# yizuo417/RollingDepth

Hardware: AMD Instinct MI355X
Metric: depth frames/sec at 768px snip_len=3, 1-step denoise; 1/2/4/8 MI355X (higher is better)
Workload: dtype f16; 1 GPU; fast preset: 100-frame 768x768 video, dilations [1, 25] (cap_dilation=True), snippet_len 3, 1-step DDIM, aligner 2000 it, refine 0; SD2-shaped UNet+VAE random-init; preset=fast, frames=100, res=768, parallelism=snippet-dp1

## Files before the change

### include/rdmi.h

```cpp
#ifndef RDMI_H
#define RDMI_H

#include <stddef.h>

#ifdef __cplusplus
extern "C" {
#endif

#define RDMI_OK 0
#define RDMI_E_ARG 1001
#define RDMI_E_ALIGN 1002
#define RDMI_E_UNSUPPORTED 1003

#define RDMI_F16 0
#define RDMI_F32 1
#define RDMI_U8 2
#define RDMI_F32_X3 3
#define RDMI_F32_X6 4

#define RDMI_RESIZE_NEAREST 0
#define RDMI_RESIZE_BILINEAR 1
#define RDMI_RESIZE_BICUBIC 2

#define RDMI_EPI_NONE 0
#define RDMI_EPI_GEGLU 1
#define RDMI_EPI_SILU 2

const char* rdmi_last_error(void);
int rdmi_version(void);

typedef struct rdmi_gemm_args {
  const void* A; long lda; long strideA;
  const void* W; long ldw; long strideW;
  void* C; long ldc; long strideC; int c_f32;
  const float* bias;
  const void* residual; long ldr; long strideR;
  const float* rowbias; int rows_per_group; long rowbias_ld;
  float alpha;
  int M, N, K, batch;
  int epilogue;
  float* gn_part; long gn_ld;
  int dtype;
} rdmi_gemm_args;
int rdmi_gemm(const rdmi_gemm_args* args, void* stream);

typedef struct rdmi_conv_args {
  const void* x; const void* w; void* y;
  const float* bias; const void* residual; const float* rowbias;
  int B, H, W, Cin, Cout, kh, kw, stride, pad_top, pad_left, upsample, Ho, Wo, Kp;
  long y_ld; long res_ld; float alpha; long rowbias_ld;
  float* gn_part; long gn_ld;
  const float* in_mean_rstd; const float* in_gamma; const float* in_beta; int in_groups, in_silu;
  int dtype;
  const void* w_up2;
  const float* in_affine;
} rdmi_conv_args;
int rdmi_conv2d(const rdmi_conv_args* args, void* stream);
int rdmi_conv2d_in_gn_supported(const rdmi_conv_args* args);

long rdmi_groupnorm_workspace(int B, int G);
int rdmi_groupnorm_stats(const void* x, int dtype, int B, long HW, int C, int G, float eps,
                         float* mean_rstd, float* workspace, void* stream);
int rdmi_groupnorm_stats_partials(const float* part, long part_ld, int B, long HW, int C, int G, float eps,
                                  float* mean_rstd, void* stream);
int rdmi_groupnorm_affine(const float* mean_rstd, const float* gamma, const float* beta, int B, int C, int G,
                          float* out, void* stream);
int rdmi_groupnorm_apply(const void* x, void* y, int dtype, int B, long HW, int C, int G,
                         const float* mean_rstd, const float* gamma, const float* beta, int silu,
                         void* stream);

long rdmi_conv3x3_to1_gn_workspace(int B, int H, int W);
int rdmi_conv3x3_to1_gn(const void* x, int dtype, int B, int H, int W, int C, int G, const float* mean_rstd,
                        const float* gamma, const float* beta, int silu, const float* w, float bias,
                        void* y, int y_dtype, float* workspace, void* stream);

int rdmi_layernorm(const void* x, void* y, int dtype, long M, int C, const float* gamma, const float* beta,
                   float eps, void* stream);

int rdmi_attention_fwd(const void* q, const void* k, const void* v, void* o, int B, int H, int Sq,
                       int Sk, int D, long q_ld, long k_ld, long v_ld, long o_ld, long q_bs,
                       long k_bs, long v_bs, long o_bs, float scale, int dtype, void* stream);

int rdmi_attention_smallkv(const void* q, const void* k, const void* v, void* o, int B, int H,
                           int Sq, int L, int D, long q_ld, long o_ld, long q_bs, long o_bs,
                           long kv_bs, float scale, int dtype, void* stream);

int rdmi_cross_attn_pair(const void* x, void* y, long M, int C, int H, const float* ln_gamma,
                         const float* ln_beta, float eps, const float* w, const float* u, const float* c,
                         void* stream);

int rdmi_softmax_rows(const float* s, void* p, long rows, long cols, long p_ld, float scale, int p_dtype,
                      void* stream);

int rdmi_nchw_to_nhwc(const void* x, int x_f32, void* y, int y_dtype, int B, int C, int H, int W, int Cpad,
                      float scale, long x_bstride, long x_cstride, void* stream);
int rdmi_nhwc_to_nchw_f32(const void* x, int dtype, long ld, float* y, int B, int C, int H, int W,
                          float scale, float shift, void* stream);
int rdmi_concat_channels(const void* a, int Ca, const void* b, int Cb, void* y, long P, int dtype, void* stream);
int rdmi_resize_nearest(const void* x, int B, int H, int W, int C, void* y, int Ho, int Wo, int dtype,
                        void* stream);
int rdmi_transpose(const void* src, void* dst, int batch, long rows, long cols, long src_ld,
                   long dst_ld, int dtype, void* stream);
int rdmi_gather_unet_input(const void* rgb, long rgb_frame_ld, const void* depth,
                           long depth_frame_ld, int depth_bcast, const int* frame_idx, int count,
                           long HW, void* out, int dtype, void* stream);
int rdmi_ddim_combine(const void* x, long ld_x, const void* e, long ld_e, void* y, long ld_y,
                      long P, int C, int Cpad, float ca, float cb, float out_scale, long e_period,
                      int dtype, void* stream);
int rdmi_snippet_average(const void* src, int n, int w, int stride, int N, long P, int C, int ld,
                         void* out, int dtype, void* stream);
int rdmi_colorize(const void* depth, int dtype, long n, const void* minmax, const unsigned char* lut, int lut_n,
                  unsigned char* rgb, int* index, void* stream);
int rdmi_snippet_accumulate(const void* src, int dtype, int k0, int nloc, int w, int stride, int N, long P, int C,
                            int ld, double* sum, void* stream);
int rdmi_snippet_finish(const double* sum, int n, int w, int stride, int N, long P, int C, int ld, void* out,
                        int dtype, void* stream);
int rdmi_snippet_average_strided(const void* src, int n, int w, int stride, int start_step, int N, long P, int C,
                                 int ld, void* out, int dtype, void* stream);
int rdmi_snippet_accumulate_strided(const void* src, int dtype, int k0, int nloc, int w, int stride, int start_step,
                                    int N, long P, int C, int ld, double* sum, void* stream);
int rdmi_snippet_finish_strided(const double* sum, int n, int w, int stride, int start_step, int N, long P, int C,
                                int ld, void* out, int dtype, void* stream);
int rdmi_minmax(const void* x, int x_f32, long n, float* minmax, float* workspace, void* stream);
int rdmi_renormalize_f32(float* x, long n, const float* minmax, void* stream);

typedef struct rdmi_aligner_args {
  int n_dil;
// ... 139 lines not shown
```

### rollingdepth_amd/_native.py

```python
from __future__ import annotations

import ctypes as C
import os

_LIB_PATH = os.environ.get("RDMI_LIB") or os.path.join(os.path.dirname(os.path.abspath(__file__)), "_lib", "librdmi.so")

vp = C.c_void_p
i32 = C.c_int
i64 = C.c_long
f32 = C.c_float


class GemmArgs(C.Structure):
    _fields_ = [
        ("A", vp), ("lda", i64), ("strideA", i64),
        ("W", vp), ("ldw", i64), ("strideW", i64),
        ("C", vp), ("ldc", i64), ("strideC", i64), ("c_f32", i32),
        ("bias", vp),
        ("residual", vp), ("ldr", i64), ("strideR", i64),
        ("rowbias", vp), ("rows_per_group", i32), ("rowbias_ld", i64),
        ("alpha", f32),
        ("M", i32), ("N", i32), ("K", i32), ("batch", i32),
        ("epilogue", i32),
        ("gn_part", vp), ("gn_ld", i64),
        ("dtype", i32),
    ]


class ConvArgs(C.Structure):
    _fields_ = [
        ("x", vp), ("w", vp), ("y", vp),
        ("bias", vp), ("residual", vp), ("rowbias", vp),
        ("B", i32), ("H", i32), ("W", i32), ("Cin", i32), ("Cout", i32), ("kh", i32), ("kw", i32),
        ("stride", i32), ("pad_top", i32), ("pad_left", i32), ("upsample", i32), ("Ho", i32), ("Wo", i32),
        ("Kp", i32),
        ("y_ld", i64), ("res_ld", i64), ("alpha", f32), ("rowbias_ld", i64),
        ("gn_part", vp), ("gn_ld", i64),
        ("in_mean_rstd", vp), ("in_gamma", vp), ("in_beta", vp), ("in_groups", i32), ("in_silu", i32),
        ("dtype", i32),
        ("w_up2", vp),
        ("in_affine", vp),
    ]


class AlignerArgs(C.Structure):
    _fields_ = [
        ("n_dil", i32),
        ("x", vp * 8), ("s", vp * 8), ("t", vp * 8),
        ("n", i32 * 8), ("stride", i32 * 8),
        ("w", i32 * 8), ("seq_len", i32), ("P", i64),
        ("lr", f32), ("beta1", f32), ("beta2", f32), ("eps", f32), ("lmda2", f32), ("lmda3", f32),
        ("depth_w", f32), ("loss_scale", f32),
        ("iters", i32),
        ("history", vp), ("workspace", vp),
        ("start_step", i32 * 8),
    ]


_SIGS = {
    "rdmi_last_error": (C.c_char_p, []),
    "rdmi_version": (i32, []),
    "rdmi_gemm": (i32, [C.POINTER(GemmArgs), vp]),
    "rdmi_conv2d": (i32, [C.POINTER(ConvArgs), vp]),
    "rdmi_conv2d_in_gn_supported": (i32, [C.POINTER(ConvArgs)]),
    "rdmi_groupnorm_workspace": (i64, [i32, i32]),
    "rdmi_groupnorm_stats": (i32, [vp, i32, i32, i64, i32, i32, f32, vp, vp, vp]),
    "rdmi_groupnorm_stats_partials": (i32, [vp, i64, i32, i64, i32, i32, f32, vp, vp]),
    "rdmi_groupnorm_apply": (i32, [vp, vp, i32, i32, i64, i32, i32, vp, vp, vp, i32, vp]),
    "rdmi_conv3x3_to1_gn_workspace": (i64, [i32, i32, i32]),
    "rdmi_conv3x3_to1_gn": (i32, [vp, i32, i32, i32, i32, i32, i32, vp, vp, vp, i32, vp, f32, vp, i32, vp, vp]),
    "rdmi_layernorm": (i32, [vp, vp, i32, i64, i32, vp, vp, f32, vp]),
    "rdmi_attention_fwd": (i32, [vp, vp, vp, vp, i32, i32, i32, i32, i32, i64, i64, i64, i64, i64, i64, i64, i64,
                                 f32, i32, vp]),
    "rdmi_attention_smallkv": (i32, [vp, vp, vp, vp, i32, i32, i32, i32, i32, i64, i64, i64, i64, i64, f32, i32, vp]),
    "rdmi_cross_attn_pair": (i32, [vp, vp, i64, i32, i32, vp, vp, f32, vp, vp, vp, vp]),
    "rdmi_softmax_rows": (i32, [vp, vp, i64, i64, i64, f32, i32, vp]),
    "rdmi_nchw_to_nhwc": (i32, [vp, i32, vp, i32, i32, i32, i32, i32, i32, f32, i64, i64, vp]),
    "rdmi_nhwc_to_nchw_f32": (i32, [vp, i32, i64, vp, i32, i32, i32, i32, f32, f32, vp]),
    "rdmi_concat_channels": (i32, [vp, i32, vp, i32, vp, i64, i32, vp]),
    "rdmi_resize_nearest": (i32, [vp, i32, i32, i32, i32, vp, i32, i32, i32, vp]),
    "rdmi_transpose": (i32, [vp, vp, i32, i64, i64, i64, i64, i32, vp]),
    "rdmi_gather_unet_input": (i32, [vp, i64, vp, i64, i32, vp, i32, i64, vp, i32, vp]),
    "rdmi_ddim_combine": (i32, [vp, i64, vp, i64, vp, i64, i64, i32, i32, f32, f32, f32, i64, i32, vp]),
    "rdmi_snippet_average": (i32, [vp, i32, i32, i32, i32, i64, i32, i32, vp, i32, vp]),
    "rdmi_snippet_accumulate": (i32, [vp, i32, i32, i32, i32, i32, i32, i64, i32, i32, vp, vp]),
    "rdmi_snippet_finish": (i32, [vp, i32, i32, i32, i32, i64, i32, i32, vp, i32, vp]),
    "rdmi_snippet_average_strided": (i32, [vp, i32, i32, i32, i32, i32, i64, i32, i32, vp, i32, vp]),
    "rdmi_snippet_accumulate_strided": (i32, [vp, i32, i32, i32, i32, i32, i32, i32, i64, i32, i32, vp, vp]),
    "rdmi_snippet_finish_strided": (i32, [vp, i32, i32, i32, i32, i32, i64, i32, i32, vp, i32, vp]),
    "rdmi_colorize": (i32, [vp, i32, i64, vp, vp, i32, vp, vp, vp]),
    "rdmi_resize_workspace": (C.c_size_t, [i32, i32, i32, i32, i32, i32]),
    "rdmi_attention_d512": (i32, [vp, vp, vp, vp, i32, i32, i32, i32] + [i64] * 8 + [C.c_float, vp, vp]),
    "rdmi_resize": (i32, [vp, i32, i64, i64, i64, i64, i32, i32, i32, i32, i32, i32, i32, i32, vp, vp, vp]),
    "rdmi_minmax": (i32, [vp, i32, i64, vp, vp, vp]),
    "rdmi_renormalize_f32": (i32, [vp, i64, vp, vp]),
    "rdmi_aligner_workspace": (i64, [C.POINTER(AlignerArgs)]),
    "rdmi_aligner_optimize": (i32, [C.POINTER(AlignerArgs), vp]),
    "rdmi_aligner_prepare": (i32, [vp, i32, i32, i32, i32, i32, i32, i32, vp, vp, vp]),
    "rdmi_aligner_merge": (i32, [i32, C.POINTER(vp), i32, C.POINTER(vp), C.POINTER(vp), C.POINTER(i32),
                                 C.POINTER(i32), C.POINTER(i32), i32, i64, vp, vp, vp]),
    "rdmi_aligner_merge_strided": (i32, [i32, C.POINTER(vp), i32, C.POINTER(vp), C.POINTER(vp), C.POINTER(i32),
                                         C.POINTER(i32), C.POINTER(i32), C.POINTER(i32), i32, i64, vp, vp, vp]),
    "rdmi_groupnorm_affine": (i32, [vp, vp, vp, i32, i32, i32, vp, vp]),
    "rdmi_aligner_merge_partial_window": (i32, [i32, C.POINTER(vp), i32, C.POINTER(vp), C.POINTER(vp),
                                                C.POINTER(i32), C.POINTER(i32), C.POINTER(i32), C.POINTER(i32),
                                                C.POINTER(i32), i32, i32, i64, vp, vp, vp]),
    "rdmi_aligner_merge_finish_pieces": (i32, [i32, C.POINTER(i32), C.POINTER(i32), C.POINTER(i32), i32, i32, i64,
                                               i32, C.POINTER(i32), C.POINTER(i32), vp, vp, vp]),
    "rdmi_aligner_merge_partial_window_strided": (i32, [i32, C.POINTER(vp), i32, C.POINTER(vp), C.POINTER(vp),
                                                        C.POINTER(i32), C.POINTER(i32), C.POINTER(i32),
                                                        C.POINTER(i32), C.POINTER(i32), C.POINTER(i32), i32, i32, i32,
                                                        i64, vp, vp, vp]),
    "rdmi_aligner_merge_finish_pieces_strided": (i32, [i32, C.POINTER(i32), C.POINTER(i32), C.POINTER(i32),
                                                       C.POINTER(i32), i32, i32, i32, i64, i32, C.POINTER(i32),
                                                       C.POINTER(i32), vp, vp, vp]),
    "rdmi_aligner_merge_moments": (i32, [i32, C.POINTER(vp), i32, C.POINTER(vp), C.POINTER(vp), C.POINTER(i32),
                                         C.POINTER(i32), C.POINTER(i32), C.POINTER(i32), i32, i64, vp, vp, vp, vp]),
    "rdmi_aligner_merge_partial_window_moments": (i32, [i32, C.POINTER(vp), i32, C.POINTER(vp), C.POINTER(vp),
                                                        C.POINTER(i32), C.POINTER(i32), C.POINTER(i32),
                                                        C.POINTER(i32), C.POINTER(i32), C.POINTER(i32), i32, i32, i32,
                                                        i64, vp, vp, vp]),
    "rdmi_aligner_merge_finish_pieces_moments": (i32, [i32, C.POINTER(i32), C.POINTER(i32), C.POINTER(i32),
                                                       C.POINTER(i32), i32, i32, i32, i64, i32, C.POINTER(i32),
                                                       C.POINTER(i32), vp, vp, vp, vp]),
    "rdmi_scale_spread_f32": (i32, [vp, i64, vp, vp]),
    "rdmi_aligner_merge_median": (i32, [i32, C.POINTER(vp), i32, C.POINTER(vp), C.POINTER(vp), C.POINTER(i32),
                                        C.POINTER(i32), C.POINTER(i32), C.POINTER(i32), i32, i64, vp, vp, vp, vp]),
    "rdmi_aligner_merge_partial_window_terms": (i32, [i32, C.POINTER(vp), i32, C.POINTER(vp), C.POINTER(vp),
                                                      C.POINTER(i32), C.POINTER(i32), C.POINTER(i32),
                                                      C.POINTER(i32), C.POINTER(i32), C.POINTER(i32), i32, i32, i32,
                                                      i64, vp, vp, i64, vp, vp]),
    "rdmi_aligner_median_rows": (i32, [vp, i64, vp, vp, i32, i64, i32, vp, vp, vp]),
    "rdmi_depth_metrics_workspace": (i64, [i32, i64]),
    "rdmi_depth_moments": (i32, [vp, i32, vp, i32, vp, i32, i64, f32, f32, vp, vp]),
    "rdmi_depth_fit": (i32, [vp, i32, i64, i32, vp, vp, vp]),
    "rdmi_depth_errors": (i32, [vp, i32, vp, i32, vp, i32, i64, f32, f32, vp, f32, f32, vp, vp, vp]),
    "rdmi_depth_moments_space": (i32, [vp, i32, vp, i32, vp, i32, i64, f32, f32, i32, vp, vp]),
    "rdmi_depth_errors_space": (i32, [vp, i32, vp, i32, vp, i32, i64, f32, f32, vp, i32, f32, f32, vp, vp, vp]),
    "rdmi_depth_temporal": (i32, [vp, i32, vp, i32, vp, vp, vp, i32, i32, i32, i32, f32, f32, vp, i32, f32, f32, vp,
                                  vp, vp]),
    "rdmi_select_bins": (i32, []),
    "rdmi_select_passes": (i32, []),
    "rdmi_select_state_bytes": (i64, []),
    "rdmi_quantiles_workspace": (i64, []),
    "rdmi_select_hist": (i32, [vp, i32, vp, i64, vp, i32, i32, vp, vp]),
# ... 47 lines not shown
```

### rollingdepth_amd/csrc/conv_occ2.hip

```cpp
#include "gemm_kernels.h"

namespace rdmi_gk {

template <int MODE>
static void occ2_mode_launch(bool gn, bool pipe, dim3 g, hipStream_t s, const GemmP& p) {
  if (gn && pipe)
    hipLaunchKernelGGL((conv_halo_occ2_kernel<MODE, true, true>), g, dim3(256), 0, s, p);
  else if (gn)
    hipLaunchKernelGGL((conv_halo_occ2_kernel<MODE, true, false>), g, dim3(256), 0, s, p);
  else if (pipe)
    hipLaunchKernelGGL((conv_halo_occ2_kernel<MODE, false, true>), g, dim3(256), 0, s, p);
  else
    hipLaunchKernelGGL((conv_halo_occ2_kernel<MODE, false, false>), g, dim3(256), 0, s, p);
}

void launch_conv_occ2(int mode, bool gn, bool pipe, dim3 g, hipStream_t s, const GemmP& p) {
  if (mode == 3) {
    if (pipe)
      hipLaunchKernelGGL((conv_halo_occ2_kernel<3, false, true>), g, dim3(256), 0, s, p);
    else
      hipLaunchKernelGGL((conv_halo_occ2_kernel<3, false, false>), g, dim3(256), 0, s, p);
  } else if (mode == 2)
    occ2_mode_launch<2>(gn, pipe, g, s, p);
  else
    occ2_mode_launch<1>(gn, pipe, g, s, p);
}

void launch_conv_h32(bool gn, dim3 g, hipStream_t s, const GemmP& p) {
  if (gn)
    hipLaunchKernelGGL((conv_halo32_kernel<true>), g, dim3(256), 0, s, p);
  else
    hipLaunchKernelGGL((conv_halo32_kernel<false>), g, dim3(256), 0, s, p);
}

void launch_gemm_occ2(int bn, dim3 g, hipStream_t s, const GemmP& p) {
  if (bn == 160 && !p.geglu)
    hipLaunchKernelGGL((gemm_occ2_kernel<0, 160>), g, dim3(256), 0, s, p);
  else
    hipLaunchKernelGGL((gemm_occ2_kernel<0, 128>), g, dim3(256), 0, s, p);
}

}
```

### rollingdepth_amd/csrc/gemm.hip

```cpp
#include "gemm_kernels.h"

#include <stdlib.h>

namespace {

using namespace rdmi_gk;


int occ2_mode() {
  const char* e = getenv("RDMI_GEMM_OCC2");
  return e ? atoi(e) : 1;
}

int pp_mode() {
  const char* e = getenv("RDMI_GEMM_PP");
  return e ? atoi(e) : 1;
}

double tile_cost(long tiles, int bm, int bn, double eff) {
  return (double)((tiles + 255) / 256) * bm * bn / eff;
}

template <int MODE, int WM, int RN>
void launch_pp(const GemmP& p, int batch, hipStream_t s) {
  constexpr int BM = WM * 128, BN = (8 / WM) * RN * 16;
  dim3 g(p.N / BN, rdmi::div_up(p.M, BM), batch);
  static_assert(RN == 4, "ping-pong tiles use RN = 4");
  launch_gemm_pp(MODE, WM, 0, g, s, p);
}

template <int MODE>
void launch_mode(const GemmP& p, int batch, hipStream_t s, bool force128) {
  if (MODE == 0) {
    const int oc = occ2_mode();
    const bool pick = !p.geglu && batch == 1 && !p.c_f32 && p.N <= 1920 && p.N % 128 != 0;
    if (oc == 2 || (oc == 1 && pick)) {
      const char* e160 = getenv("RDMI_GEMM_BN160");
      const int bn = (p.N % 160 == 0 && !p.geglu && !(e160 && e160[0] == '0')) ? 160 : 128;
      dim3 g(rdmi::div_up(p.N, bn), rdmi::div_up(p.M, 128), batch);
      launch_gemm_occ2(bn, g, s, p);
      return;
    }
  }
  const int pp = pp_mode();
  if (pp != 0 && (MODE == 0 || p.cmaj)) {
    const char* dbg = MODE == 0 ? getenv("RDMI_GEMM_DBG") : nullptr;
    if (dbg && p.N % 256 == 0) {
      dim3 g(p.N / 256, rdmi::div_up(p.M, 256), batch);
      const int dv = atoi(dbg);
      if (dv == 1 || dv == 5 || dv == 8 || dv == 12) {
        launch_gemm_pp(0, 2, dv, g, s, p);
        return;
      }
    }
    const long mt256 = rdmi::div_up(p.M, 256), mt512 = rdmi::div_up(p.M, 512);
    const long ct = rdmi::div_up(p.N, 128);
    const double classic = tile_cost(mt256 * ct * batch, 256, 128, 1.0);
    double best = pp == 2 ? 1e300 : classic;
    int pick = 0;
    if (p.N % 256 == 0) {
      const double c = tile_cost(mt256 * (p.N / 256) * batch, 256, 256, 1.3);
      if (c < best) best = c, pick = 1;
    }
    if (p.N % 128 == 0) {
      const double c = tile_cost(mt512 * (p.N / 128) * batch, 512, 128, 1.1);
      if (c < best) best = c, pick = 3;
    }
    switch (pick) {
      case 1: launch_pp<MODE, 2, 4>(p, batch, s); return;
      case 3: launch_pp<MODE, 4, 4>(p, batch, s); return;
      default: break;
    }
  }
  const long mt256 = (p.M + 255) / 256;
  if (force128 || p.N % 128 == 0 || p.N > 512) {
    if (mt256 * ((p.N + 127) / 128) * batch >= 512) {
      dim3 g(rdmi::div_up(p.N, 128), rdmi::div_up(p.M, 256), batch);
      launch_gemm_classic(MODE, 256, 128, g, s, p);
    } else {
      dim3 g(rdmi::div_up(p.N, 128), rdmi::div_up(p.M, 128), batch);
      launch_gemm_classic(MODE, 128, 128, g, s, p);
    }
  } else {
    dim3 g(rdmi::div_up(p.N, 64), rdmi::div_up(p.M, 256), batch);
    launch_gemm_classic(MODE, 256, 64, g, s, p);
  }
}

int launch(GemmP p, int batch, hipStream_t s, bool force128, int mode) {
  const char* gm = getenv("RDMI_GEMM_GROUP");
  p.group_m = gm ? atoi(gm) : 8;
  if (mode == 2)
    launch_mode<2>(p, batch, s, force128);
  else if (mode == 1)
    launch_mode<1>(p, batch, s, force128);
  else
    launch_mode<0>(p, batch, s, force128);
  return rdmi::check_launch("gemm");
}

bool al16(const void* p) { return ((uintptr_t)p & 15) == 0; }

bool vec_ok(const GemmP& p) {
  const uintptr_t csz = p.c_f32 ? 16 : 8;
  bool ok = p.ldc % 4 == 0 && p.sC % 4 == 0 && ((uintptr_t)p.C % csz) == 0;
  if (p.R) ok = ok && p.ldr % 4 == 0 && p.sR % 4 == 0 && ((uintptr_t)p.R & 7) == 0;
  if (p.bias) ok = ok && ((uintptr_t)p.bias & 15) == 0;
  if (p.rowbias) ok = ok && ((uintptr_t)p.rowbias & 15) == 0 && p.rb_ld % 4 == 0;
  return ok;
}

int halo_mode() {
  const char* he = getenv("RDMI_CONV_HALO");
  return he ? atoi(he) : 3;
}

bool halo_eligible(const rdmi_conv_args* a, int hmode) {
  return hmode != 0 && a->kh == 3 && a->kw == 3 && a->Cin % 64 == 0 && a->stride == 1 && a->pad_top == 1 &&
         a->pad_left == 1 && a->Ho % 16 == 0 && a->Wo % 16 == 0 && a->Cout % 64 == 0 &&
         a->Ho == (a->upsample ? 2 * a->H : a->H) && a->Wo == (a->upsample ? 2 * a->W : a->W);
}

bool in_gn_ok(const rdmi_conv_args* a) {
  const int cmax = a->in_affine ? (1 << 30) : (a->Cout % 256 == 0 || a->Cout == 128) ? 1024 : 256;
  return a->in_groups > 0 && a->Cin <= cmax && a->Cin % a->in_groups == 0;
}

bool h32_ok(const rdmi_conv_args* a, const GemmP& p, bool gn) {
  const char* e = getenv("RDMI_CONV_H32");
  if (!e || e[0] != '1') return false;
  return !a->upsample && a->Cout % 128 == 0 && a->Cin % 128 == 0 && a->Ho % 8 == 0 && a->Wo % 32 == 0 && p.vec && !p.c_f32 &&
         ((uintptr_t)p.C & 15) == 0 && p.ldc % 8 == 0 && (!p.R || (((uintptr_t)p.R & 15) == 0 && p.ldr % 8 == 0)) &&
         (!p.bias || ((uintptr_t)p.bias & 15) == 0) && (!gn || a->Cin <= 256);
}

bool conv1x1_ok(const GemmP& p) {
  const char* e = getenv("RDMI_CONV1X1");
  if (e && e[0] == '0') return false;
  return !p.R && !p.rowbias && !p.gnp && p.vec && ((uintptr_t)p.C & 15) == 0 && p.ldc % 8 == 0 && p.ldw % 8 == 0 &&
         (!p.bias || ((uintptr_t)p.bias & 15) == 0);
}

}

extern "C" int rdmi_conv2d_in_gn_supported(const rdmi_conv_args* a) {
  return a && a->dtype == RDMI_F16 && halo_eligible(a, halo_mode()) && in_gn_ok(a) ? 1 : 0;
}

extern "C" int rdmi_gemm(const rdmi_gemm_args* a, void* stream) {
  RDMI_REQUIRE(a && a->A && a->W && a->C, RDMI_E_ARG, "gemm: null pointer");
  RDMI_REQUIRE(a->M > 0 && a->N > 0 && a->K > 0 && a->batch > 0, RDMI_E_ARG, "gemm: bad sizes M=%d N=%d K=%d", a->M, a->N, a->K);
  RDMI_REQUIRE(a->dtype == RDMI_F16 || a->dtype == RDMI_F32 || a->dtype == RDMI_F32_X3 || a->dtype == RDMI_F32_X6,
               RDMI_E_UNSUPPORTED, "gemm: dtype %d", a->dtype);
  if (a->dtype != RDMI_F16) return rdmi::gemm_f32(a, stream);
  RDMI_REQUIRE(a->K % 8 == 0 && a->lda % 8 == 0 && a->ldw % 8 == 0 && a->ldw >= a->K,
               RDMI_E_ALIGN, "gemm: K (%d), lda (%ld) must be multiples of 8 and ldw (%ld) >= K", a->K, a->lda, a->ldw);
  RDMI_REQUIRE(al16(a->A) && al16(a->W) && a->strideA % 8 == 0 && a->strideW % 8 == 0, RDMI_E_ALIGN, "gemm: A/W not 16-byte aligned");
  RDMI_REQUIRE(a->epilogue != RDMI_EPI_GEGLU || a->N % 128 == 0, RDMI_E_ARG, "gemm: GEGLU needs N %% 128 == 0");
  RDMI_REQUIRE(!a->rowbias || a->rows_per_group > 0, RDMI_E_ARG, "gemm: rowbias needs rows_per_group");
  RDMI_REQUIRE((long)a->M * a->lda < (1L << 30) && (long)a->N * a->ldw < (1L << 30), RDMI_E_ARG,
               "gemm: operand exceeds 2^30 elements (2 GiB) per batch");
  GemmP p{};
  p.A = (const f16*)a->A; p.lda = a->lda; p.sA = a->strideA;
  p.Wt = (const f16*)a->W; p.ldw = a->ldw; p.sW = a->strideW;
  p.C = a->C; p.ldc = a->ldc; p.sC = a->strideC; p.c_f32 = a->c_f32;
  p.bias = a->bias; p.R = (const f16*)a->residual; p.ldr = a->ldr; p.sR = a->strideR;
  p.rowbias = a->rowbias; p.rpg = a->rows_per_group > 0 ? a->rows_per_group : 1; p.rb_ld = a->rowbias_ld;
  p.alpha = a->alpha;
  p.M = a->M; p.N = a->N; p.K = (a->K + BK - 1) / BK * BK; p.Kvalid = a->K;
  p.geglu = a->epilogue == RDMI_EPI_GEGLU;
  p.silu = a->epilogue == RDMI_EPI_SILU;
  p.vec = vec_ok(p);
  RDMI_REQUIRE(!p.geglu || p.vec, RDMI_E_ALIGN, "gemm: GEGLU output needs 4-element aligned rows");
  p.gnp = a->gn_part; p.gn_ld = a->gn_ld;
  RDMI_REQUIRE(!p.gnp || (a->batch == 1 && !p.c_f32 && !p.geglu && p.vec && a->N % 4 == 0 && a->M % 32 == 0 &&
                          ((uintptr_t)p.gnp & 7) == 0 && p.gn_ld >= 2L * (a->M / 32)),
               RDMI_E_ARG, "gemm: GroupNorm moments need batch 1, f16 vector output, N %% 4 == 0, M %% 32 == 0");
  p.a_bytes = (unsigned)(((long)(a->M - 1) * a->lda + a->K) * 2);
  p.w_bytes = (unsigned)(((long)(a->N - 1) * a->ldw + a->K) * 2);
  return launch(p, a->batch, (hipStream_t)stream, p.geglu, 0);
}

extern "C" int rdmi_conv2d(const rdmi_conv_args* a, void* stream) {
  RDMI_REQUIRE(a && a->x && a->w && a->y, RDMI_E_ARG, "conv2d: null pointer");
  RDMI_REQUIRE(a->B > 0 && a->H > 0 && a->W > 0 && a->Cout > 0 && a->Ho > 0 && a->Wo > 0, RDMI_E_ARG, "conv2d: bad sizes");
  RDMI_REQUIRE(a->dtype == RDMI_F16 || a->dtype == RDMI_F32 || a->dtype == RDMI_F32_X3 || a->dtype == RDMI_F32_X6,
               RDMI_E_UNSUPPORTED, "conv2d: dtype %d", a->dtype);
  if (a->dtype != RDMI_F16) return rdmi::conv2d_f32(a, stream);
  RDMI_REQUIRE(a->Cin % 8 == 0, RDMI_E_ALIGN, "conv2d: Cin (%d) must be a multiple of 8", a->Cin);
  const int K = a->kh * a->kw * a->Cin;
  RDMI_REQUIRE(a->Kp >= K && a->Kp % 8 == 0, RDMI_E_ARG, "conv2d: Kp (%d) must be >= %d and a multiple of 8", a->Kp, K);
  RDMI_REQUIRE(al16(a->x) && al16(a->w), RDMI_E_ALIGN, "conv2d: x/w not 16-byte aligned");
  RDMI_REQUIRE((long)a->B * a->H * a->W * a->Cin < (1L << 30) && (long)a->Cout * a->Kp < (1L << 30), RDMI_E_ARG,
               "conv2d: input exceeds 2^30 elements (2 GiB; split the batch)");
  GemmP p{};
  p.A = (const f16*)a->x; p.Wt = (const f16*)a->w; p.ldw = a->Kp;
  p.C = a->y; p.ldc = a->y_ld > 0 ? a->y_ld : a->Cout;
  p.bias = a->bias; p.R = (const f16*)a->residual; p.ldr = a->res_ld > 0 ? a->res_ld : a->Cout;
  p.rowbias = a->rowbias; p.rpg = a->Ho * a->Wo; p.rb_ld = a->rowbias_ld;
  p.alpha = a->alpha;
  p.M = a->B * a->Ho * a->Wo; p.N = a->Cout; p.K = a->Kp; p.Kvalid = K;
  p.IH = a->H; p.IW = a->W; p.Cin = a->Cin; p.Ho = a->Ho; p.Wo = a->Wo;
  p.kh = a->kh; p.kw = a->kw; p.stride = a->stride; p.pt = a->pad_top; p.pl = a->pad_left;
  p.up = a->upsample ? 1 : 0; p.cin_vecs = a->Cin / 8;
  p.cmaj = a->kh * a->kw > 1 && a->Cin % 64 == 0;
  const bool dense = a->kh == 1 && a->kw == 1 && a->stride == 1 && a->pad_top == 0 && a->pad_left == 0 && !a->upsample &&
                     a->Ho == a->H && a->Wo == a->W;
  if (dense) p.lda = a->Cin;
  RDMI_REQUIRE(dense || (a->kh == 3 && a->kw == 3), RDMI_E_UNSUPPORTED, "conv2d: only 3x3 and dense 1x1 kernels");
  RDMI_REQUIRE(!a->upsample || a->stride == 1, RDMI_E_UNSUPPORTED, "conv2d: upsample needs stride 1");
  p.vec = vec_ok(p);
  p.gnp = a->gn_part; p.gn_ld = a->gn_ld;
  RDMI_REQUIRE(!p.gnp || (p.vec && a->Cout % 4 == 0 && p.M % 32 == 0 && ((uintptr_t)p.gnp & 7) == 0 &&
                          p.gn_ld >= 2L * (p.M / 32)),
               RDMI_E_ARG, "conv2d: GroupNorm moments need vector output, Cout %% 4 == 0, B*Ho*Wo %% 32 == 0");
  p.a_bytes = (unsigned)((long)a->B * a->H * a->W * a->Cin * 2);
  p.w_bytes = (unsigned)((long)a->Cout * a->Kp * 2);
  const int hmode = halo_mode();
  RDMI_REQUIRE(!a->in_mean_rstd || (a->in_gamma && a->in_beta), RDMI_E_ARG, "conv2d: input GroupNorm needs gamma and beta");
  RDMI_REQUIRE(!a->in_mean_rstd || (halo_eligible(a, hmode) && in_gn_ok(a)), RDMI_E_UNSUPPORTED,
               "conv2d: input GroupNorm not supported for this shape (rdmi_conv2d_in_gn_supported)");
  if (halo_eligible(a, hmode)) {
    const char* gm = getenv("RDMI_GEMM_GROUP");
    p.group_m = gm ? atoi(gm) : 8;
    const char* nx = getenv("RDMI_CONV_NXCD");
    if (nx && nx[0] == '1') p.group_m = -1;
    const char* cpp = getenv("RDMI_CONV_PIPE");
    p.conv_pipe = !cpp || cpp[0] != '0';
    const char* hpf = getenv("RDMI_HALO_PREF");
    p.halo_pref = hpf && hpf[0] == '1';
// ... 43 lines not shown
```

### rollingdepth_amd/csrc/gemm_kernels.h

```cpp
#pragma once
#include "common.h"

#include <utility>

namespace rdmi_gk {

constexpr int BK = 64;

struct GemmP {
  const f16* A; long lda, sA;
  const f16* Wt; long ldw, sW;
  void* C; long ldc, sC; int c_f32;
  const float* bias;
  const f16* R; long ldr, sR;
  const float* rowbias; int rpg; long rb_ld;
  float alpha;
  int M, N, K, Kvalid;
  int geglu, silu, vec;
  unsigned a_bytes, w_bytes;
  int IH, IW, Cin, Ho, Wo, kh, kw, stride, pt, pl, up, cin_vecs;
  int cmaj;
  float* gnp; long gn_ld;
  int group_m;
  const float* gmr; const float* ggam; const float* gbet; int gG, gsilu;
  const float* gaff;
  int cperm;
  int conv_pipe;
  int halo_pref;
  int xprio;
  int eprio;
  unsigned long long* stamps;
};

__device__ __forceinline__ unsigned long long gk_stamp() {
  unsigned long long t;
  __builtin_amdgcn_sched_barrier(0);
  asm volatile("s_memtime %0\n\ts_waitcnt lgkmcnt(0)" : "=s"(t) :: "memory");
  __builtin_amdgcn_sched_barrier(0);
  return t;
}

template <int N>
__device__ __forceinline__ void wait_vmcnt() {
  __builtin_amdgcn_s_waitcnt((N & 0xF) | (((N >> 4) & 3) << 14) | (0x7 << 4) | (0xF << 8));
}

constexpr unsigned OOB = 0x80000000u;

__device__ __forceinline__ f16x4 gn_pack4(const float* f, bool in) {
  unsigned w0, w1;
  asm("v_cvt_pk_f16_f32 %0, %1, %2" : "=v"(w0) : "v"(f[0]), "v"(f[1]));
  asm("v_cvt_pk_f16_f32 %0, %1, %2" : "=v"(w1) : "v"(f[2]), "v"(f[3]));
  if (!__all(in)) {
    w0 = in ? w0 : 0u;
    w1 = in ? w1 : 0u;
  }
  return __builtin_bit_cast(f16x4, (__attribute__((ext_vector_type(2))) unsigned){w0, w1});
}

template <bool HI>
__device__ __forceinline__ float gn_elem(unsigned w, float sc, float sh) {
  float f;
  if (HI)
    asm("v_fma_mix_f32 %0, %1, %2, %3 op_sel:[1,0,0] op_sel_hi:[1,0,0]" : "=v"(f) : "v"(w), "v"(sc), "v"(sh));
  else
    asm("v_fma_mix_f32 %0, %1, %2, %3 op_sel_hi:[1,0,0]" : "=v"(f) : "v"(w), "v"(sc), "v"(sh));
  return f;
}

__device__ __forceinline__ void silu4(float (&f)[4]) {
  float t0, t1, t2, t3;
  asm("v_mul_f32 %0, 0xbfb8aa3b, %4\n\t"
      "v_mul_f32 %1, 0xbfb8aa3b, %5\n\t"
      "v_mul_f32 %2, 0xbfb8aa3b, %6\n\t"
      "v_mul_f32 %3, 0xbfb8aa3b, %7\n\t"
      "v_exp_f32 %0, %0\n\t"
      "v_exp_f32 %1, %1\n\t"
      "v_exp_f32 %2, %2\n\t"
      "v_exp_f32 %3, %3\n\t"
      "v_add_f32 %0, 1.0, %0\n\t"
      "v_add_f32 %1, 1.0, %1\n\t"
      "v_add_f32 %2, 1.0, %2\n\t"
      "v_add_f32 %3, 1.0, %3\n\t"
      "v_rcp_f32 %0, %0\n\t"
      "v_rcp_f32 %1, %1\n\t"
      "v_rcp_f32 %2, %2\n\t"
      "v_rcp_f32 %3, %3\n\t"
      "v_mul_f32 %0, %4, %0\n\t"
      "v_mul_f32 %1, %5, %1\n\t"
      "v_mul_f32 %2, %6, %2\n\t"
      "v_mul_f32 %3, %7, %3"
      : "=&v"(t0), "=&v"(t1), "=&v"(t2), "=&v"(t3)
      : "v"(f[0]), "v"(f[1]), "v"(f[2]), "v"(f[3]));
  f[0] = t0;
  f[1] = t1;
  f[2] = t2;
  f[3] = t3;
}

template <int NW, bool SILU>
__device__ __forceinline__ void gn_xform_words(unsigned (&w)[NW], const float* sc, const float* sh, bool in) {
#pragma unroll
  for (int j = 0; j < NW; j += 2) {
    float f[4] = {gn_elem<false>(w[j], sc[2 * j], sh[2 * j]), gn_elem<true>(w[j], sc[2 * j + 1], sh[2 * j + 1]),
                  gn_elem<false>(w[j + 1], sc[2 * j + 2], sh[2 * j + 2]),
                  gn_elem<true>(w[j + 1], sc[2 * j + 3], sh[2 * j + 3])};
    if (SILU) silu4(f);
    const f16x4 o = gn_pack4(f, in);
    const auto u = __builtin_bit_cast(__attribute__((ext_vector_type(2))) unsigned, o);
    w[j] = u[0];
    w[j + 1] = u[1];
  }
}

__device__ __forceinline__ void dma16(__amdgpu_buffer_rsrc_t r, unsigned voff, f16* l) {
  __builtin_amdgcn_raw_ptr_buffer_load_lds(r, (__attribute__((address_space(3))) void*)l, 16, voff, 0, 0, 0);
}
__device__ __forceinline__ void dma16s(__amdgpu_buffer_rsrc_t r, unsigned voff, int soff, f16* l) {
  __builtin_amdgcn_raw_ptr_buffer_load_lds(r, (__attribute__((address_space(3))) void*)l, 16, voff, soff, 0, 0);
}

template <int CTRL>
__device__ __forceinline__ float dpp_f(float v) {
  return __builtin_bit_cast(float, __builtin_amdgcn_update_dpp(0, __builtin_bit_cast(int, v), CTRL, 0xF, 0xF, false));
}
__device__ __forceinline__ float row16_sum(float v) {
  v += dpp_f<0xB1>(v);
  v += dpp_f<0x4E>(v);
  v += dpp_f<0x141>(v);
  v += dpp_f<0x140>(v);
  return v;
}

struct LinRows {
  int mw, fr, M;
  __device__ int row(int i) const {
    const int m = mw + i * 16 + fr;
    return m < M ? m : -1;
  }
  __device__ long slot(int i) const { return (mw + (i - 1) * 16) >> 5; }
  __device__ bool full(int n) const { return mw + n * 16 <= M; }
  __device__ int group(int n, int rpg) const { return mw / rpg == (mw + n * 16 - 1) / rpg ? mw / rpg : -1; }
  __device__ int rstep() const { return 16; }
};
struct PatchRows {
  int b, Ho, Wo, y0, x0, rw, fr;
  __device__ int row(int i) const { return (b * Ho + y0 + rw + i) * Wo + x0 + fr; }
  __device__ long slot(int i) const { return (long)((b * Ho + y0 + rw + i - 1) >> 1) * (Wo >> 4) + (x0 >> 4); }
  __device__ bool full(int) const { return true; }
  __device__ int group(int, int rpg) const { return rpg == Ho * Wo ? b : -1; }
  __device__ int rstep() const { return Wo; }
};
struct PhaseRows {
  int b, Ho, Wo, y0, x0, rw, fr, a, c;
  __device__ int row(int i) const { return (b * Ho + 2 * (y0 + rw + i) + a) * Wo + 2 * (x0 + fr) + c; }
  __device__ long slot(int i) const {
    return (long)(b * 4 + 2 * a + c) * ((Ho >> 1) * (Wo >> 1) >> 5) + ((y0 + rw + i - 1) >> 1) * (Wo >> 5) + (x0 >> 4);
  }
  __device__ bool full(int) const { return true; }
  __device__ int group(int, int rpg) const { return rpg == Ho * Wo ? b : -1; }
  __device__ int rstep() const { return 2 * Wo; }
};

__device__ __forceinline__ int perm64(int r) {
  const int j = r >> 4, c = r & 15;
  return 32 * (j >> 1) + 8 * (c >> 2) + 4 * (j & 1) + (c & 3);
}
__device__ __forceinline__ int col_base(bool perm, int nw, int j, int fq) {
  return perm ? nw + 32 * (j >> 1) + 8 * fq + 4 * (j & 1) : nw + j * 16 + fq * 4;
}

template <int RM, int RN, int WTN, bool SILU, class Rows>
__device__ __forceinline__ void store_tile_t(const GemmP& p, f32x4 (&acc)[RM][RN], const Rows& rows, int nw, int bz,
                                             int fr, int fq, bool perm) {
  const long cb = (long)bz * p.sC;
  const long rbz = (long)bz * p.sR;
  const int rbg = p.rowbias ? rows.group(RM, p.rpg) : 0;
  if (!p.geglu && !p.c_f32 && p.vec && rows.full(RM) && nw + RN * 16 <= p.N && rbg >= 0) {
    f32x4 bb[RN], rbv[RN];
    if (p.bias) {
#pragma unroll
      for (int j = 0; j < RN; ++j) bb[j] = *(const f32x4*)(p.bias + col_base(perm, nw, j, fq));
    } else {
#pragma unroll
      for (int j = 0; j < RN; ++j) bb[j] = f32x4{0.f, 0.f, 0.f, 0.f};
    }
    if (p.rowbias) {
      const float* rbp = p.rowbias + (long)rbg * p.rb_ld;
#pragma unroll
      for (int j = 0; j < RN; ++j) rbv[j] = *(const f32x4*)(rbp + col_base(perm, nw, j, fq));
    }
    f16x4 rr[RM][RN];
    if (p.R) {
#pragma unroll
      for (int i = 0; i < RM; ++i) {
        const f16* rrow = p.R + rbz + (long)rows.row(i) * p.ldr;
        if (perm && RN % 2 == 0) {
#pragma unroll
          for (int j = 0; j < RN; j += 2) {
            const f16x8 v = *(const f16x8*)(rrow + col_base(true, nw, j, fq));
            rr[i][j] = __builtin_shufflevector(v, v, 0, 1, 2, 3);
            rr[i][j + 1] = __builtin_shufflevector(v, v, 4, 5, 6, 7);
          }
        } else {
#pragma unroll
          for (int j = 0; j < RN; ++j) rr[i][j] = *(const f16x4*)(rrow + col_base(false, nw, j, fq));
        }
      }
    }
    f32x4 badd[RN];
#pragma unroll
    for (int j = 0; j < RN; ++j) badd[j] = p.rowbias ? bb[j] + rbv[j] : bb[j];
    float gs[RN], gq[RN];
#pragma unroll
    for (int i = 0; i < RM; ++i) {
      const long crow = cb + (long)rows.row(i) * p.ldc;
      f16x4 ov[RN];
#pragma unroll
      for (int j = 0; j < RN; ++j) {
        const int n = col_base(perm, nw, j, fq);
        f16x4 o;
        float s = 0.f, q = 0.f;
#pragma unroll
        for (int r = 0; r < 4; ++r) {
          float v = acc[i][j][r] * p.alpha + badd[j][r];
          if (p.R) v += (float)rr[i][j][r];
          if constexpr (SILU) v = silu_f(v);
// ... 1510 lines not shown
            q += dpp_f<0x142>(q);
            if ((lane & 31) == 16) {
              float* d = p.gnp + (long)((nb + 4 * g) >> 2) * p.gn_ld + slot * 2;
              *(__attribute__((ext_vector_type(2))) float*)d = {s, q};
            }
          }
        }
      }
    }
  };
  auto epilogue = [&](auto RESc, auto SILUc) {
    constexpr bool RES = decltype(RESc)::value, SILU = decltype(SILUc)::value;
#pragma unroll
    for (int c = 0; c < 2; ++c) {
      const int nb = n0 + 64 * wn + 32 * c + 16 * hh;
      f32x4 badd[4];
#pragma unroll
      for (int q = 0; q < 4; ++q) {
        badd[q] = p.bias ? *(const f32x4*)(p.bias + nb + 4 * q) : f32x4{0.f, 0.f, 0.f, 0.f};
        if (p.rowbias) badd[q] += *(const f32x4*)(p.rowbias + rbg + nb + 4 * q);
      }
      f16x8 rr[4][2];
      if constexpr (RES) {
#pragma unroll
        for (int pb = 0; pb < 4; ++pb) {
          const long m = (long)(b * p.Ho + y0 + 4 * wm + pb) * p.Wo + x0 + j;
          const f16* rrow = p.R + m * p.ldr + nb;
          rr[pb][0] = *(const f16x8*)rrow;
          rr[pb][1] = *(const f16x8*)(rrow + 8);
        }
      }
#pragma unroll
      for (int pb = 0; pb < 4; ++pb) {
        const long m = (long)(b * p.Ho + y0 + 4 * wm + pb) * p.Wo + x0 + j;
        f16x8 ov[2];
        float gs[4], gq[4];
#pragma unroll
        for (int i = 0; i < 16; ++i) {
          float v = acc[pb][c][i] * p.alpha + badd[i >> 2][i & 3];
          if constexpr (RES) v += (float)rr[pb][i >> 3][i & 7];
          if constexpr (SILU) v = silu_f(v);
          const f16 o = (f16)v;
          ov[i >> 3][i & 7] = o;
          const float f = (float)o;
          if ((i & 3) == 0) {
            gs[i >> 2] = f;
            gq[i >> 2] = f * f;
          } else {
            gs[i >> 2] += f;
            gq[i >> 2] = fmaf(f, f, gq[i >> 2]);
          }
        }
        f16* crow = (f16*)p.C + m * p.ldc + nb;
        *(f16x8*)crow = ov[0];
        *(f16x8*)(crow + 8) = ov[1];
        if (p.gnp) {
          const long slot = ((long)(b * p.Ho + y0 + 4 * wm + pb) * p.Wo + x0) >> 5;
#pragma unroll
          for (int g = 0; g < 4; ++g) {
            float s = row16_sum(gs[g]), q = row16_sum(gq[g]);
            s += dpp_f<0x142>(s);
            q += dpp_f<0x142>(q);
            if ((lane & 31) == 16) {
              float* d = p.gnp + (long)((nb + 4 * g) >> 2) * p.gn_ld + slot * 2;
              d[0] = s;
              d[1] = q;
            }
          }
        }
      }
    }
  };
  using T_ = std::true_type;
  using F_ = std::false_type;
  if (p.silu) {
    if (p.R) epilogue(T_{}, T_{}); else epilogue(F_{}, T_{});
  } else if (p.R) {
    if (p.gnp) epi_fast(T_{}, T_{}); else epi_fast(T_{}, F_{});
  } else {
    if (p.gnp) epi_fast(F_{}, T_{}); else epi_fast(F_{}, F_{});
  }
}

template <int V = 0, int BN = 128>
__global__ __launch_bounds__(256, 2) void gemm_occ2_kernel(GemmP p) {
  constexpr int BM = 128, BKP = 64, RM = 4, RN = BN / 32, WN = BN / 2;
  constexpr int NA = 4, NB = BN / 32;
  constexpr int SLOT = (BM + BN) * BKP;
  __shared__ __attribute__((aligned(16))) f16 lds[2 * SLOT];

  const int tid = threadIdx.x;
  const int lane = tid & 63;
  const int wid = tid >> 6;
  const int wids = __builtin_amdgcn_readfirstlane(wid);
  const int wm = wid >> 1, wn = wid & 1;
  const int nbx = gridDim.x;
  const int logical = xcd_remap(blockIdx.y * nbx + blockIdx.x, nbx * gridDim.y);
  int mt_, nt_;
  tile_mn(logical, nbx, gridDim.y, p.group_m, mt_, nt_);
  const int n0 = nt_ * BN, m0 = mt_ * BM;
  const int bz = blockIdx.z;
  const __amdgpu_buffer_rsrc_t ra_ =
      __builtin_amdgcn_make_buffer_rsrc((void*)(p.A + (long)bz * p.sA), (short)0, (int)p.a_bytes, 0x00020000);
  const __amdgpu_buffer_rsrc_t rw_ =
      __builtin_amdgcn_make_buffer_rsrc((void*)(p.Wt + (long)bz * p.sW), (short)0, (int)p.w_bytes, 0x00020000);

  const int lrow = lane >> 3;
  const int chunk = (lane & 7) ^ lrow;
  unsigned avo[NA], bvo[NB];
#pragma unroll
  for (int e = 0; e < NA; ++e) {
    const int m = m0 + (wid + 4 * e) * 8 + lrow;
    avo[e] = m < p.M ? (unsigned)(m * (int)p.lda + chunk * 8) * 2u : OOB;
  }
#pragma unroll
  for (int e = 0; e < NB; ++e) {
    const int n = n0 + (wid + 4 * e) * 8 + lrow;
    bvo[e] = n < p.N ? (unsigned)(n * (int)p.ldw + chunk * 8) * 2u : OOB;
  }
  auto issue = [&](int u) {
    const bool kok = u * BKP + chunk * 8 < p.Kvalid;
    f16* la = lds + (u & 1) * SLOT;
    f16* lb = la + BM * BKP;
#pragma unroll
    for (int e = 0; e < NA; ++e) dma16s(ra_, kok ? avo[e] : OOB, u * BKP * 2, la + (wids + 4 * e) * 8 * BKP);
#pragma unroll
    for (int e = 0; e < NB; ++e) dma16s(rw_, kok ? bvo[e] : OOB, u * BKP * 2, lb + (wids + 4 * e) * 8 * BKP);
  };

  f32x4 acc[RM][RN];
#pragma unroll
  for (int i = 0; i < RM; ++i)
#pragma unroll
    for (int j = 0; j < RN; ++j) acc[i][j] = f32x4{0.f, 0.f, 0.f, 0.f};

  const int nk = (p.K + BKP - 1) / BKP;
  const int fr = lane & 15, fq = lane >> 4;
  const int off0 = fr * BKP + ((fq ^ (fr & 7)) << 3);
  const int off1 = fr * BKP + (((4 + fq) ^ (fr & 7)) << 3);

  const bool live = n0 + (wids & 1) * WN < p.N;
  issue(0);
  wait_vmcnt<0>();
  asm volatile("" ::: "memory");
  __builtin_amdgcn_s_barrier();
  asm volatile("" ::: "memory");
  for (int u = 0; u < nk; ++u) {
    if (u > 0) {
      wait_vmcnt<0>();
      asm volatile("s_waitcnt lgkmcnt(0)" ::: "memory");
      __builtin_amdgcn_s_barrier();
      asm volatile("" ::: "memory");
    }
    if (u + 1 < nk) issue(u + 1);
    if (!live) continue;
    const f16* la = lds + (u & 1) * SLOT + (wm * 64) * BKP;
    const f16* lb = lds + (u & 1) * SLOT + BM * BKP + (wn * WN) * BKP;
    f16x8 af[2][RM], bf[2][RN];
#pragma unroll
    for (int kh = 0; kh < 2; ++kh) {
      const int off = kh ? off1 : off0;
#pragma unroll
      for (int j = 0; j < RN; ++j) bf[kh][j] = *(const f16x8*)(lb + j * 16 * BKP + off);
#pragma unroll
      for (int i = 0; i < RM; ++i) af[kh][i] = *(const f16x8*)(la + i * 16 * BKP + off);
    }
#pragma unroll
    for (int kh = 0; kh < 2; ++kh)
#pragma unroll
      for (int i = 0; i < RM; ++i)
#pragma unroll
        for (int j = 0; j < RN; ++j)
          acc[i][j] = __builtin_amdgcn_mfma_f32_16x16x32_f16(bf[kh][j], af[kh][i], acc[i][j], 0, 0, 0);
  }
  if (live) store_tile<RM, RN, WN>(p, acc, LinRows{m0 + wm * 64, fr, p.M}, n0 + wn * WN, bz, fr, fq);
}

void launch_gemm_classic(int mode, int bm, int bn, dim3 g, hipStream_t s, const GemmP& p);
void launch_gemm_pp(int mode, int wm, int dbg, dim3 g, hipStream_t s, const GemmP& p);
void launch_gemm_occ2(int bn, dim3 g, hipStream_t s, const GemmP& p);
void launch_conv_halo(int mode, int nph, int wn, bool gn, dim3 g, hipStream_t s, const GemmP& p);
void launch_conv_occ2(int mode, bool gn, bool pipe, dim3 g, hipStream_t s, const GemmP& p);
void launch_conv_h32(bool gn, dim3 g, hipStream_t s, const GemmP& p);
bool launch_conv1x1(const GemmP& p, int cin, int cout, hipStream_t st);

}
```

### rollingdepth_amd/csrc/runtime.cpp

```cpp
#include "common.h"

#include <string.h>

namespace rdmi {

static thread_local char g_err[512] = "";

void set_error(const char* fmt, ...) {
  va_list ap;
  va_start(ap, fmt);
  vsnprintf(g_err, sizeof(g_err), fmt, ap);
  va_end(ap);
}

int check_launch(const char* what) {
  hipError_t e = hipGetLastError();
  if (e != hipSuccess) {
    set_error("%s: launch failed: %s", what, hipGetErrorString(e));
    return (int)e;
  }
  return 0;
}

}

extern "C" const char* rdmi_last_error(void) { return rdmi::g_err; }
extern "C" int rdmi_version(void) { return 11; }
```

Baseline: 23.72 depth frames/s.

## Split GEMM tail wave into smaller occ2 tiles to balance CU load

When the ping-pong 256-row GEMM grid leaves a partial last wave across CUs, the M range is split. The head rows run with the large ping-pong kernel for whole waves and the remainder runs as a second launch of the 128x128 occupancy-2 kernel with an M offset, including an implicit-conv addressing path for conv modes. The aim is to cut wave-quantization idle time on the tail. The cost is an extra launch, new kernel template instantiations, and a heuristic cost model that decides when to split.

```diff
diff --git a/include/rdmi.h b/include/rdmi.h
--- a/include/rdmi.h
+++ b/include/rdmi.h
@@ -43,6 +43,7 @@
   int dtype;
 } rdmi_gemm_args;
 int rdmi_gemm(const rdmi_gemm_args* args, void* stream);
+long rdmi_gemm_tail_splits(void);
 
 typedef struct rdmi_conv_args {
   const void* x; const void* w; void* y;
diff --git a/rollingdepth_amd/_native.py b/rollingdepth_amd/_native.py
--- a/rollingdepth_amd/_native.py
+++ b/rollingdepth_amd/_native.py
@@ -61,6 +61,7 @@
     "rdmi_last_error": (C.c_char_p, []),
     "rdmi_version": (i32, []),
     "rdmi_gemm": (i32, [C.POINTER(GemmArgs), vp]),
+    "rdmi_gemm_tail_splits": (i64, []),
     "rdmi_conv2d": (i32, [C.POINTER(ConvArgs), vp]),
     "rdmi_conv2d_in_gn_supported": (i32, [C.POINTER(ConvArgs)]),
     "rdmi_groupnorm_workspace": (i64, [i32, i32]),
diff --git a/rollingdepth_amd/csrc/conv_occ2.hip b/rollingdepth_amd/csrc/conv_occ2.hip
--- a/rollingdepth_amd/csrc/conv_occ2.hip
+++ b/rollingdepth_amd/csrc/conv_occ2.hip
@@ -33,7 +33,16 @@
     hipLaunchKernelGGL((conv_halo32_kernel<false>), g, dim3(256), 0, s, p);
 }
 
-void launch_gemm_occ2(int bn, dim3 g, hipStream_t s, const GemmP& p) {
+void launch_gemm_occ2(int bn, dim3 g, hipStream_t s, const GemmP& p, int mode, bool tail) {
+  if (mode != 0 || tail) {
+    if (mode == 1)
+      hipLaunchKernelGGL((gemm_occ2_kernel<0, 128, 1, true>), g, dim3(256), 0, s, p);
+    else if (mode == 2)
+      hipLaunchKernelGGL((gemm_occ2_kernel<0, 128, 2, true>), g, dim3(256), 0, s, p);
+    else
+      hipLaunchKernelGGL((gemm_occ2_kernel<0, 128, 0, true>), g, dim3(256), 0, s, p);
+    return;
+  }
   if (bn == 160 && !p.geglu)
     hipLaunchKernelGGL((gemm_occ2_kernel<0, 160>), g, dim3(256), 0, s, p);
   else
diff --git a/rollingdepth_amd/csrc/gemm.hip b/rollingdepth_amd/csrc/gemm.hip
--- a/rollingdepth_amd/csrc/gemm.hip
+++ b/rollingdepth_amd/csrc/gemm.hip
@@ -1,6 +1,9 @@
 #include "gemm_kernels.h"
+#include "tail_split.h"
 
 #include <stdlib.h>
+
+#include <atomic>
 
 namespace {
 
@@ -29,8 +32,35 @@
   launch_gemm_pp(MODE, WM, 0, g, s, p);
 }
 
+int cu_count() {
+  static int cus[64] = {};
+  int dev = 0;
+  if (hipGetDevice(&dev) != hipSuccess || dev < 0 || dev >= 64) return 256;
+  if (cus[dev] == 0) {
+    int n = 0;
+    cus[dev] = hipDeviceGetAttribute(&n, hipDeviceAttributeMultiprocessorCount, dev) == hipSuccess && n > 0 ? n : 256;
+  }
+  return cus[dev];
+}
+
+std::atomic<long> g_tail_splits{0};
+
 template <int MODE>
-void launch_mode(const GemmP& p, int batch, hipStream_t s, bool force128) {
+bool launch_tail_split(const GemmP& p, int batch, hipStream_t s, bool any_depth) {
+  if (!any_depth && !rdmi_tail::tail_depth_ok(MODE == 0, p.Kvalid)) return false;
+  if (batch != 1 || p.geglu || p.silu || p.c_f32 || p.alpha != 1.0f) return false;
+  const rdmi_tail::TailPlan t = rdmi_tail::plan_tail_split(p.M, 256, p.N / 256, batch, cu_count(), rdmi_tail::Q_PP256);
+  if (t.m_split == 0) return false;
+  launch_gemm_pp(MODE, 2, 0, dim3(p.N / 256, t.head_rows, 1), s, p);
+  GemmP q = p;
+  q.m_off = t.m_split;
+  launch_gemm_occ2(128, dim3(p.N / 128, rdmi::div_up(p.M - t.m_split, rdmi_tail::TAIL_BM), 1), s, q, MODE, true);
+  g_tail_splits.fetch_add(1, std::memory_order_relaxed);
+  return true;
+}
+
+template <int MODE>
+void launch_mode(const GemmP& p, int batch, hipStream_t s, bool force128, int tail) {
   if (MODE == 0) {
     const int oc = occ2_mode();
     const bool pick = !p.geglu && batch == 1 && !p.c_f32 && p.N <= 1920 && p.N % 128 != 0;
@@ -67,7 +97,10 @@
       if (c < best) best = c, pick = 3;
     }
     switch (pick) {
-      case 1: launch_pp<MODE, 2, 4>(p, batch, s); return;
+      case 1:
+        if (tail && launch_tail_split<MODE>(p, batch, s, tail == 2)) return;
+        launch_pp<MODE, 2, 4>(p, batch, s);
+        return;
       case 3: launch_pp<MODE, 4, 4>(p, batch, s); return;
       default: break;
     }
@@ -90,12 +123,14 @@
 int launch(GemmP p, int batch, hipStream_t s, bool force128, int mode) {
   const char* gm = getenv("RDMI_GEMM_GROUP");
   p.group_m = gm ? atoi(gm) : 8;
+  const char* gt = getenv("RDMI_GEMM_TAIL");
+  const int tail = gt ? atoi(gt) : 1;
   if (mode == 2)
-    launch_mode<2>(p, batch, s, force128);
+    launch_mode<2>(p, batch, s, force128, tail);
   else if (mode == 1)
-    launch_mode<1>(p, batch, s, force128);
+    launch_mode<1>(p, batch, s, force128, tail);
   else
-    launch_mode<0>(p, batch, s, force128);
+    launch_mode<0>(p, batch, s, force128, tail);
   return rdmi::check_launch("gemm");
 }
 
@@ -146,6 +181,8 @@
 extern "C" int rdmi_conv2d_in_gn_supported(const rdmi_conv_args* a) {
   return a && a->dtype == RDMI_F16 && halo_eligible(a, halo_mode()) && in_gn_ok(a) ? 1 : 0;
 }
+
+extern "C" long rdmi_gemm_tail_splits(void) { return g_tail_splits.load(std::memory_order_relaxed); }
 
 extern "C" int rdmi_gemm(const rdmi_gemm_args* a, void* stream) {
   RDMI_REQUIRE(a && a->A && a->W && a->C, RDMI_E_ARG, "gemm: null pointer");
diff --git a/rollingdepth_amd/csrc/gemm_kernels.h b/rollingdepth_amd/csrc/gemm_kernels.h
--- a/rollingdepth_amd/csrc/gemm_kernels.h
+++ b/rollingdepth_amd/csrc/gemm_kernels.h
@@ -22,6 +22,7 @@
   int cmaj;
   float* gnp; long gn_ld;
   int group_m;
+  int m_off;
   const float* gmr; const float* ggam; const float* gbet; int gG, gsilu;
   const float* gaff;
   int cperm;
@@ -143,6 +144,13 @@
   __device__ int group(int n, int rpg) const { return mw / rpg == (mw + n * 16 - 1) / rpg ? mw / rpg : -1; }
   __device__ int rstep() const { return 16; }
 };
+struct TailRows : LinRows {
+  __device__ bool full(int) const { return (mw & ~127) + 128 <= M; }
+  __device__ int group(int, int rpg) const {
+    const int pm = mw & ~127;
+    return pm / rpg == (pm + 127) / rpg ? pm / rpg : -1;
+  }
+};
 struct PatchRows {
   int b, Ho, Wo, y0, x0, rw, fr;
   __device__ int row(int i) const { return (b * Ho + y0 + rw + i) * Wo + x0 + fr; }
@@ -1819,7 +1827,7 @@
   }
 }
 
-template <int V = 0, int BN = 128>
+template <int V = 0, int BN = 128, int MODE = 0, bool TAIL = false>
 __global__ __launch_bounds__(256, 2) void gemm_occ2_kernel(GemmP p) {
   constexpr int BM = 128, BKP = 64, RM = 4, RN = BN / 32, WN = BN / 2;
   constexpr int NA = 4, NB = BN / 32;
@@ -1835,7 +1843,7 @@
   const int logical = xcd_remap(blockIdx.y * nbx + blockIdx.x, nbx * gridDim.y);
   int mt_, nt_;
   tile_mn(logical, nbx, gridDim.y, p.group_m, mt_, nt_);
-  const int n0 = nt_ * BN, m0 = mt_ * BM;
+  const int n0 = nt_ * BN, m0 = mt_ * BM + p.m_off;
   const int bz = blockIdx.z;
   const __amdgpu_buffer_rsrc_t ra_ =
       __builtin_amdgcn_make_buffer_rsrc((void*)(p.A + (long)bz * p.sA), (short)0, (int)p.a_bytes, 0x00020000);
@@ -1845,11 +1853,27 @@
   const int lrow = lane >> 3;
   const int chunk = (lane & 7) ^ lrow;
   unsigned avo[NA], bvo[NB];
+  int arow[NA], ahb[NA], awb[NA];
 #pragma unroll
   for (int e = 0; e < NA; ++e) {
     const int m = m0 + (wid + 4 * e) * 8 + lrow;
-    avo[e] = m < p.M ? (unsigned)(m * (int)p.lda + chunk * 8) * 2u : OOB;
-  }
+    const bool ok = m < p.M;
+    if (MODE == 0) {
+      avo[e] = ok ? (unsigned)(m * (int)p.lda + chunk * 8) * 2u : OOB;
+    } else {
+      const int mm = ok ? m : 0;
+      const int hw = p.Ho * p.Wo;
+      const int b = mm / hw;
+      const int r = mm - b * hw;
+      const int ho = r / p.Wo;
+      const int wo = r - ho * p.Wo;
+      const int hb = ho * p.stride - p.pt;
+      ahb[e] = ok ? hb : -(1 << 28);
+      awb[e] = wo * p.stride - p.pl;
+      arow[e] = MODE == 1 ? (b * p.IH + hb) * p.IW * p.Cin + awb[e] * p.Cin : b * p.IH * p.IW * p.Cin;
+    }
+  }
+  const int Hl = p.IH << (MODE == 2 ? 1 : 0), Wl = p.IW << (MODE == 2 ? 1 : 0);
 #pragma unroll
   for (int e = 0; e < NB; ++e) {
     const int n = n0 + (wid + 4 * e) * 8 + lrow;
@@ -1859,8 +1883,28 @@
     const bool kok = u * BKP + chunk * 8 < p.Kvalid;
     f16* la = lds + (u & 1) * SLOT;
     f16* lb = la + BM * BKP;
-#pragma unroll
-    for (int e = 0; e < NA; ++e) dma16s(ra_, kok ? avo[e] : OOB, u * BKP * 2, la + (wids + 4 * e) * 8 * BKP);
+    if (MODE == 0) {
+#pragma unroll
+      for (int e = 0; e < NA; ++e) dma16s(ra_, kok ? avo[e] : OOB, u * BKP * 2, la + (wids + 4 * e) * 8 * BKP);
+    } else {
+      const int cb = u / 9;
+      const int tap = u - cb * 9;
+      const int dy = (tap * 11) >> 5, dx = tap - 3 * dy;
+      const bool cok = cb * 64 < p.Cin;
+      const int cofs = cb * 64 + chunk * 8;
+      const int tapoff = (dy * p.IW + dx) * p.Cin + cofs;
+#pragma unroll
+      for (int e = 0; e < NA; ++e) {
+        const int hi = ahb[e] + dy, wi = awb[e] + dx;
+        const bool ok = cok && (unsigned)hi < (unsigned)Hl && (unsigned)wi < (unsigned)Wl;
+        int off;
+        if (MODE == 1)
+          off = arow[e] + tapoff;
+        else
+          off = arow[e] + ((hi >> 1) * p.IW + (wi >> 1)) * p.Cin + cofs;
+        dma16(ra_, ok ? (unsigned)off * 2u : OOB, la + (wids + 4 * e) * 8 * BKP);
+      }
+    }
 #pragma unroll
     for (int e = 0; e < NB; ++e) dma16s(rw_, kok ? bvo[e] : OOB, u * BKP * 2, lb + (wids + 4 * e) * 8 * BKP);
   };
@@ -1910,12 +1954,17 @@
         for (int j = 0; j < RN; ++j)
           acc[i][j] = __builtin_amdgcn_mfma_f32_16x16x32_f16(bf[kh][j], af[kh][i], acc[i][j], 0, 0, 0);
   }
-  if (live) store_tile<RM, RN, WN>(p, acc, LinRows{m0 + wm * 64, fr, p.M}, n0 + wn * WN, bz, fr, fq);
+  if (!live) return;
+  const LinRows rows{m0 + wm * 64, fr, p.M};
+  if constexpr (TAIL)
+    store_tile<RM, RN, WN>(p, acc, TailRows{rows}, n0 + wn * WN, bz, fr, fq);
+  else
+    store_tile<RM, RN, WN>(p, acc, rows, n0 + wn * WN, bz, fr, fq);
 }
 
 void launch_gemm_classic(int mode, int bm, int bn, dim3 g, hipStream_t s, const GemmP& p);
 void launch_gemm_pp(int mode, int wm, int dbg, dim3 g, hipStream_t s, const GemmP& p);
-void launch_gemm_occ2(int bn, dim3 g, hipStream_t s, const GemmP& p);
+void launch_gemm_occ2(int bn, dim3 g, hipStream_t s, const GemmP& p, int mode = 0, bool tail = false);
 void launch_conv_halo(int mode, int nph, int wn, bool gn, dim3 g, hipStream_t s, const GemmP& p);
 void launch_conv_occ2(int mode, bool gn, bool pipe, dim3 g, hipStream_t s, const GemmP& p);
 void launch_conv_h32(bool gn, dim3 g, hipStream_t s, const GemmP& p);
diff --git a/rollingdepth_amd/csrc/runtime.cpp b/rollingdepth_amd/csrc/runtime.cpp
--- a/rollingdepth_amd/csrc/runtime.cpp
+++ b/rollingdepth_amd/csrc/runtime.cpp
@@ -25,4 +25,4 @@
 }
 
 extern "C" const char* rdmi_last_error(void) { return rdmi::g_err; }
-extern "C" int rdmi_version(void) { return 11; }
+extern "C" int rdmi_version(void) { return 12; }
diff --git a/rollingdepth_amd/csrc/tail_split.h b/rollingdepth_amd/csrc/tail_split.h
--- /dev/null
+++ b/rollingdepth_amd/csrc/tail_split.h
@@ -0,0 +1,56 @@
+#pragma once
+
+namespace rdmi_tail {
+
+constexpr double Q_PP256 = 0.63;
+
+constexpr int MAX_DENSE_K = 1280;
+
+inline bool tail_depth_ok(bool dense, int K) { return !dense || K <= MAX_DENSE_K; }
+
+constexpr int MAX_TAIL_NTILES = 15;
+
+constexpr int TAIL_BM = 128;
+
+struct TailPlan {
+  int m_split;
+  int head_rows;
+  long head_tiles;
+  long tail_tiles;
+  double cost;
+  double unsplit;
+};
+
+inline long ceil_div(long a, long b) { return (a + b - 1) / b; }
+
+inline TailPlan plan_tail_split(long M, int bm, int n_tiles, int batch, int slots, double q) {
+  TailPlan t{};
+  if (M <= 0 || (bm != 256 && bm != 512) || n_tiles <= 0 || batch <= 0 || slots <= 0 || !(q > 0.0)) return t;
+  const long row = (long)n_tiles * batch;
+  const long mt = ceil_div(M, bm);
+  const long total = mt * row;
+  t.unsplit = t.cost = (double)ceil_div(total, slots);
+  if (total < slots) return t;
+  if (total % slots == 0) return t;
+  const long tail_n = (long)n_tiles * (512 / bm);
+  if (tail_n > MAX_TAIL_NTILES) return t;
+  const long R = total / slots;
+  const long h = R * slots / row;
+  if (h <= 0 || h >= mt) return t;
+  const long head_tiles = h * row;
+  const long head_rounds = ceil_div(head_tiles, slots);
+  if (head_rounds != R) return t;
+  const long tail_rows = M - h * bm;
+  const long tail_tiles = ceil_div(tail_rows, TAIL_BM) * tail_n * batch;
+  const long tail_rounds = ceil_div(tail_tiles, 2L * slots);
+  const double cost = (double)head_rounds + (double)tail_rounds * q;
+  if (!(cost < t.unsplit)) return t;
+  t.m_split = (int)(h * bm);
+  t.head_rows = (int)h;
+  t.head_tiles = head_tiles;
+  t.tail_tiles = tail_tiles;
+  t.cost = cost;
+  return t;
+}
+
+}
```

Result: no change. 23.75 depth frames/s (median of 6 runs) (+0.2%).
